# mdejong/MetalBT709Decoder

Hardware: AMD Instinct MI355X
Metric: Gpixel/s, 4k NV12->sRGB BGRA decode (output pixels) (higher is better)
Workload: dtype f32

## Files before the change

metalbt709decoder_amd/csrc/bt709_device.h:

```cpp
#pragma once

#include <hip/hip_runtime.h>

#include <cstdint>

#include "bt709_constants.h"
#include "bt709_kernels.h"
#include "bt709_quantise.h"
#include "bt709_stage.h"
#include "bt709_tile.h"

namespace bt709 {
namespace {

typedef uint32_t u32x4 __attribute__((ext_vector_type(4)));
typedef uint32_t u32x2 __attribute__((ext_vector_type(2)));
typedef __attribute__((address_space(3))) const u32x2 *LdsPairPtr;
typedef __attribute__((address_space(3))) const u32x4 *LdsQuadPtr;

__device__ __forceinline__ uint32_t lds_address(const void *p) {
  return static_cast<uint32_t>(reinterpret_cast<size_t>((__attribute__((address_space(3))) const unsigned char *)p));
}

__device__ __forceinline__ float byte_of(uint32_t w, int i) {
  float f = static_cast<float>((w >> (8 * i)) & 0xffu);
  asm("" : "+v"(f));
  return f;
}

__device__ __forceinline__ float byte_value(uint8_t b) {
  float f = static_cast<float>(b);
  asm("" : "+v"(f));
  return f;
}

__device__ __forceinline__ float centre_norm(float v, float off) {
  return __builtin_fmaf(v, kInv255, -off * kInv255);
}

__device__ __forceinline__ float add_sat(float a, float b) {
  float r;
  asm("v_add_f32_e64 %0, %1, %2 clamp" : "=v"(r) : "v"(a), "v"(b));
  return r;
}

struct Chroma {
  float cr_r, cb_g, cr_g, cb_b;
};

__device__ __forceinline__ Chroma chroma_terms(float cb, float cr) {
  const float cbn = centre_norm(cb, 128.0f);
  const float crn = centre_norm(cr, 128.0f);
  Chroma c;
  c.cr_r = __fmul_rn(crn, kMCrR);
  c.cb_g = __fmul_rn(cbn, kMCbG);
  c.cr_g = __fmul_rn(crn, kMCrG);
  c.cb_b = __fmul_rn(cbn, kMCbB);
  return c;
}

__device__ __forceinline__ void pixel_rgb(float ybyte, const Chroma &c, float &r, float &g, float &b) {
  const float yv = __fmul_rn(centre_norm(ybyte, 16.0f), kMY);
  r = add_sat(yv, c.cr_r);
  g = add_sat(__fadd_rn(yv, c.cb_g), c.cr_g);
  b = add_sat(yv, c.cb_b);
}

__device__ __forceinline__ float alpha_value(float abyte) {
  return add_sat(__fmul_rn(centre_norm(abyte, 16.0f), kMY), 0.0f);
}

__device__ __forceinline__ uint32_t quantise_byte(float x) {
  return quantise_enumerated(x);
}

__device__ __forceinline__ void magic_index12(const float *x, uint32_t *t, float magic) {
#pragma unroll
  for (int i = 0; i < 12; ++i) t[i] = __float_as_uint(__fadd_rn(x[i], magic));
}

__device__ __forceinline__ void magic_index4(const float *x, uint32_t *t, float magic) {
#pragma unroll
  for (int i = 0; i < 4; ++i) t[i] = __float_as_uint(__fadd_rn(x[i], magic));
}

struct UnitLookup {
  float magic;
  uint32_t offset;
  uint32_t shift;
};

template <typename Params>
__device__ __forceinline__ UnitLookup unit_lookup(const Params &p, const void *lds_table) {
  UnitLookup u;
  u.magic = p.unit1_magic;
  u.offset = lds_address(lds_table) - (p.unit1_first << 3);
  u.shift = p.unit1_shift;
  return u;
}

__device__ __forceinline__ uint32_t bucket_byte(const UnitLookup &u, float x, uint32_t t) {
  const u32x2 e = *reinterpret_cast<LdsPairPtr>((t << 3) + u.offset);
  return e.y + (x >= __uint_as_float(e.x) ? 1u : 0u);
}

__device__ __forceinline__ uint32_t pack_bgra(uint32_t R, uint32_t G, uint32_t B, uint32_t alpha_word) {
  const uint32_t rg = __builtin_amdgcn_perm(R, G, 0x0c04000cu);
  return rg | B | alpha_word;
}

__device__ __forceinline__ void stage_table(void *lds, const void *src, uint32_t bytes) {
  u32x4 *d = reinterpret_cast<u32x4 *>(lds);
  const u32x4 *s = reinterpret_cast<const u32x4 *>(src);
  const uint32_t tid = threadIdx.y * blockDim.x + threadIdx.x, nthreads = blockDim.x * blockDim.y;
  const uint32_t n = bytes / 16;
  if (n <= nthreads) {
    for (uint32_t i = tid; i < n; i += nthreads) d[i] = s[i];
    return;
  }
  stage_batched<5>(d, n, tid, nthreads, [&](uint32_t i) { return s[i]; });
}

template <bool NT>
__device__ __forceinline__ void store16(uint8_t *p, u32x4 v) {
  if (NT) __builtin_nontemporal_store(v, reinterpret_cast<u32x4 *>(p));
  else *reinterpret_cast<u32x4 *>(p) = v;
}

template <bool NT>
__device__ __forceinline__ void store8(uint8_t *p, u32x2 v) {
  if (NT) __builtin_nontemporal_store(v, reinterpret_cast<u32x2 *>(p));
  else *reinterpret_cast<u32x2 *>(p) = v;
}

__device__ __forceinline__ FramePlanes frame_planes(const DecodeParams &p, uint32_t i) {
  if (!p.uniform) return p.frames[i];
  FramePlanes f = p.frames[0];
  f.y += static_cast<int64_t>(i) * p.step_y;
  f.cbcr += static_cast<int64_t>(i) * p.step_cbcr;
  if (f.alpha) f.alpha += static_cast<int64_t>(i) * p.step_alpha;
  f.out += static_cast<int64_t>(i) * p.step_out;
  return f;
}

}
}
```

metalbt709decoder_amd/csrc/bt709_kernels.hip:

```cpp
#include <hip/hip_runtime.h>

#include <cstdint>
#include <cstring>

#include "bt709_device.h"
#include "bt709_launch.h"

namespace bt709 {
namespace {

template <bool HAS_ALPHA, bool QUANT, bool LOGIDX>
__device__ __forceinline__ void decode_quad(const UnitLookup &u, uint32_t ya, uint32_t yb, uint32_t cw, uint32_t aa,
                                            uint32_t ab, uint32_t alpha_word, u32x4 &top, u32x4 &bot) {
  const Chroma c0 = chroma_terms(byte_of(cw, 0), byte_of(cw, 1));
  const Chroma c1 = chroma_terms(byte_of(cw, 2), byte_of(cw, 3));
  float x[24];
#pragma unroll
  for (int px = 0; px < 8; ++px)
    pixel_rgb(byte_of(px < 4 ? ya : yb, px & 3), (px & 2) ? c1 : c0, x[3 * px], x[3 * px + 1], x[3 * px + 2]);
  static_assert(QUANT || !HAS_ALPHA, "an alpha decoder runs the sRGB mode");
  uint32_t byte[24], al[8];
  if (QUANT) {
#pragma unroll
    for (int i = 0; i < 24; ++i) byte[i] = quantise_byte(x[i]);
  } else {
    uint32_t t[24];
    magic_index12(x, t, u.magic);
    magic_index12(x + 12, t + 12, u.magic);
    if (LOGIDX) {
#pragma unroll
      for (int i = 0; i < 24; ++i) t[i] >>= 16;
    }
#pragma unroll
    for (int i = 0; i < 24; ++i) byte[i] = bucket_byte(u, x[i], t[i]);
  }
#pragma unroll
  for (int px = 0; px < 8; ++px)
    al[px] = HAS_ALPHA ? quantise_byte(alpha_value(byte_of(px < 4 ? aa : ab, px & 3))) << 24 : alpha_word;
  top.x = pack_bgra(byte[0], byte[1], byte[2], al[0]);
  top.y = pack_bgra(byte[3], byte[4], byte[5], al[1]);
  top.z = pack_bgra(byte[6], byte[7], byte[8], al[2]);
  top.w = pack_bgra(byte[9], byte[10], byte[11], al[3]);
  bot.x = pack_bgra(byte[12], byte[13], byte[14], al[4]);
  bot.y = pack_bgra(byte[15], byte[16], byte[17], al[5]);
  bot.z = pack_bgra(byte[18], byte[19], byte[20], al[6]);
  bot.w = pack_bgra(byte[21], byte[22], byte[23], al[7]);
}

template <bool HAS_ALPHA, bool QUANT>
__device__ __forceinline__ void decode_block(const UnitLookup &u, const float y[4], float cb, float cr, const float a[4],
                                             uint32_t alpha_word, uint32_t out[4]) {
  const Chroma c = chroma_terms(cb, cr);
  float x[12];
#pragma unroll
  for (int px = 0; px < 4; ++px) pixel_rgb(y[px], c, x[3 * px], x[3 * px + 1], x[3 * px + 2]);
  if (QUANT) {
#pragma unroll
    for (int px = 0; px < 4; ++px)
      out[px] = pack_bgra(quantise_byte(x[3 * px]), quantise_byte(x[3 * px + 1]), quantise_byte(x[3 * px + 2]),
                          HAS_ALPHA ? quantise_byte(alpha_value(a[px])) << 24 : alpha_word);
    return;
  }
  uint32_t t[12];
  magic_index12(x, t, u.magic);
#pragma unroll
  for (int i = 0; i < 12; ++i) t[i] >>= u.shift;
#pragma unroll
  for (int px = 0; px < 4; ++px)
    out[px] = pack_bgra(bucket_byte(u, x[3 * px], t[3 * px]), bucket_byte(u, x[3 * px + 1], t[3 * px + 1]),
                        bucket_byte(u, x[3 * px + 2], t[3 * px + 2]), alpha_word);
}

typedef __attribute__((address_space(3))) const float *LdsFloatPtr;

struct OverLookup {
  float enc_add;
  uint32_t enc_off;
  uint32_t lin_off;
};

__device__ __forceinline__ OverLookup stage_over_tables(unsigned char *lds_raw, const DecodeParams &p) {
  stage_table(lds_raw, p.table_encode, p.table_encode_bytes);
  stage_table(lds_raw + p.table_encode_bytes, p.over_table_lin, kOverLinBytes);
  OverLookup o;
  o.enc_add = p.encode_log_add;
  o.enc_off = lds_address(lds_raw) - (p.encode_log_first << 3);
  o.lin_off = lds_address(lds_raw) + p.table_encode_bytes;
  return o;
}

__device__ __forceinline__ float over_lin(const OverLookup &o, uint32_t byte) {
  return *reinterpret_cast<LdsFloatPtr>((byte << 2) + o.lin_off);
}

__device__ __forceinline__ uint32_t over_encode(const OverLookup &o, float v) {
  const uint32_t t = __float_as_uint(__fadd_rn(v, o.enc_add)) >> 16;
  const u32x2 e = *reinterpret_cast<LdsPairPtr>((t << 3) + o.enc_off);
  return e.y + (v >= __uint_as_float(e.x) ? 1u : 0u);
}

template <int OVER>
__device__ __forceinline__ uint32_t over_pixel(const OverLookup &o, const float *colour_lin, const float *x, float abyte, uint32_t bg) {
  const uint32_t as = quantise_byte(alpha_value(abyte)), inv = 255u - as;
  const float k = __fmul_rn(static_cast<float>(inv), kInv255);
  float d[3];
  uint32_t a = 255u;
  if (OVER == kOverDestination) {
    d[0] = over_lin(o, (bg >> 16) & 0xffu);
    d[1] = over_lin(o, (bg >> 8) & 0xffu);
    d[2] = over_lin(o, bg & 0xffu);
    a = as + (inv * (bg >> 24) + 127u) / 255u;
  } else {
    d[0] = colour_lin[0], d[1] = colour_lin[1], d[2] = colour_lin[2];
  }
  uint32_t byte[3];
#pragma unroll
  for (int c = 0; c < 3; ++c)
    byte[c] = over_encode(o, add_sat(over_lin(o, quantise_byte(x[c])), __fmul_rn(k, d[c])));
  return pack_bgra(byte[0], byte[1], byte[2], a << 24);
}

template <int OVER>
__device__ __forceinline__ void over_quad(const OverLookup &o, const DecodeParams &p, uint32_t ya, uint32_t yb, uint32_t cw, uint32_t aa,
                                          uint32_t ab, const u32x4 &bt, const u32x4 &bb, u32x4 &top, u32x4 &bot) {
  const Chroma c0 = chroma_terms(byte_of(cw, 0), byte_of(cw, 1));
  const Chroma c1 = chroma_terms(byte_of(cw, 2), byte_of(cw, 3));
  const uint32_t bg[8] = {bt.x, bt.y, bt.z, bt.w, bb.x, bb.y, bb.z, bb.w};
  uint32_t w[8];
#pragma unroll
  for (int px = 0; px < 8; ++px) {
    float x[3];
    pixel_rgb(byte_of(px < 4 ? ya : yb, px & 3), (px & 2) ? c1 : c0, x[0], x[1], x[2]);
    w[px] = over_pixel<OVER>(o, p.over_lin, x, byte_of(px < 4 ? aa : ab, px & 3), bg[px]);
  }
  top.x = w[0], top.y = w[1], top.z = w[2], top.w = w[3];
  bot.x = w[4], bot.y = w[5], bot.z = w[6], bot.w = w[7];
}

}

template <bool HAS_ALPHA, bool NT, bool QUANT, bool LOGIDX = false, int OVER = kOverOff>
__device__ __forceinline__ void quads_body(const DecodeParams &p, unsigned char *lds_raw) {
  constexpr int UNROLL = kQuadsPerLane;
  const BandedWork work = banded_work<true>(p.xcd_bands, p.frames_per_band);
  const FramePlanes f = frame_planes(p, work.frame);
  const uint32_t quads = p.width >> 2;
  const uint32_t row_pairs = p.height >> 1;
  const uint32_t rp_raw = blockIdx.y * blockDim.y + __builtin_amdgcn_readfirstlane(threadIdx.y);
  const uint32_t q0 = work.tile * (blockDim.x * UNROLL) + threadIdx.x;

  static_assert(OVER == kOverOff || HAS_ALPHA, "there is nothing to composite without an alpha channel");
  TileIn<UNROLL, HAS_ALPHA, OVER == kOverDestination> in;
  in.template load<NT>(f, p, rp_raw, row_pairs, q0, quads);
  OverLookup ol = {};
  if constexpr (OVER != kOverOff) {
    ol = stage_over_tables(lds_raw, p);
    __syncthreads();
  }
  if (!QUANT) {
    stage_table(lds_raw, p.table_unit, p.table_unit_bytes);
    __syncthreads();
  }
  in.pin();

  const UnitLookup ul = unit_lookup(p, lds_raw);
  uint8_t *o0 = f.out + static_cast<size_t>(2 * min(rp_raw, row_pairs - 1)) * p.out_stride;
  uint8_t *o1 = o0 + p.out_stride;
  if constexpr (OVER != kOverOff) {
#pragma unroll
    for (int u = 0; u < UNROLL; ++u) {
      const uint32_t q = q0 + u * blockDim.x;
      u32x4 top, bot;
      over_quad<OVER>(ol, p, in.ya[u], in.yb[u], in.cw[u], in.aa[u], in.ab[u], in.da[OVER == kOverDestination ? u : 0], in.db[OVER == kOverDestination ? u : 0], top, bot);
      if (q < quads && rp_raw < row_pairs) {
        store16<NT>(o0 + 16 * q, top);
        store16<NT>(o1 + 16 * q, bot);
      }
    }
    return;
  }
#pragma unroll
  for (int u = 0; u < UNROLL; ++u) {
    const uint32_t q = q0 + u * blockDim.x;
    u32x4 top, bot;
    decode_quad<HAS_ALPHA, QUANT, LOGIDX>(ul, in.ya[u], in.yb[u], in.cw[u], HAS_ALPHA ? in.aa[u] : 0u, HAS_ALPHA ? in.ab[u] : 0u, p.alpha_word, top, bot);
    if (q < quads && rp_raw < row_pairs) {
      store16<NT>(o0 + 16 * q, top);
      store16<NT>(o1 + 16 * q, bot);
    }
  }
}

template <bool HAS_ALPHA, bool NT, bool QUANT>
__global__ void __launch_bounds__(kMaxBlockThreads)
decode_nv12_quads(const DecodeParams p) {
  extern __shared__ __attribute__((aligned(16))) unsigned char lds_raw[];
  quads_body<HAS_ALPHA, NT, QUANT>(p, lds_raw);
}

template <bool NT>
__global__ void __launch_bounds__(kMaxBlockThreads)
decode_nv12_quads_log(const DecodeParams p) {
  extern __shared__ __attribute__((aligned(16))) unsigned char lds_raw[];
  quads_body<false, NT, false, true>(p, lds_raw);
}

template <int OVER>
__global__ void __launch_bounds__(kMaxBlockThreads)
decode_nv12_quads_over(const DecodeParams p) {
  extern __shared__ __attribute__((aligned(16))) unsigned char lds_raw[];
  quads_body<true, true, true, false, OVER>(p, lds_raw);
}

template <bool HAS_ALPHA, bool QUANT>
__global__ void __launch_bounds__(kBlockThreads)
decode_nv12_blocks(const DecodeParams p) {
  extern __shared__ __attribute__((aligned(16))) unsigned char lds_raw[];
  if (!QUANT) {
    stage_table(lds_raw, p.table_unit, p.table_unit_bytes);
    __syncthreads();
  }

  const UnitLookup ul = unit_lookup(p, lds_raw);
  const FramePlanes f = frame_planes(p, blockIdx.y);
  const uint32_t bw = p.width >> 1;
  const uint32_t row_pairs = p.height >> 1;

  for (uint32_t rp = blockIdx.x; rp < row_pairs; rp += gridDim.x) {
    const uint8_t *y0 = f.y + static_cast<size_t>(2 * rp) * p.y_stride;
    const uint8_t *y1 = y0 + p.y_stride;
    const uint8_t *cc = f.cbcr + static_cast<size_t>(rp) * p.cbcr_stride;
    uint32_t *o0 = reinterpret_cast<uint32_t *>(f.out + static_cast<size_t>(2 * rp) * p.out_stride);
    uint32_t *o1 = reinterpret_cast<uint32_t *>(f.out + static_cast<size_t>(2 * rp + 1) * p.out_stride);
    for (uint32_t bx = threadIdx.x; bx < bw; bx += kBlockThreads) {
      const float y[4] = {byte_value(y0[2 * bx]), byte_value(y0[2 * bx + 1]), byte_value(y1[2 * bx]),
                          byte_value(y1[2 * bx + 1])};
      float a[4] = {0.f, 0.f, 0.f, 0.f};
      if (HAS_ALPHA) {
        const uint8_t *a0 = f.alpha + static_cast<size_t>(2 * rp) * p.alpha_stride;
        const uint8_t *a1 = a0 + p.alpha_stride;
        a[0] = byte_value(a0[2 * bx]);
        a[1] = byte_value(a0[2 * bx + 1]);
        a[2] = byte_value(a1[2 * bx]);
        a[3] = byte_value(a1[2 * bx + 1]);
      }
      uint32_t out[4];
      decode_block<HAS_ALPHA, QUANT>(ul, y, byte_value(cc[2 * bx]), byte_value(cc[2 * bx + 1]), a, p.alpha_word, out);
      o0[2 * bx] = out[0];
      o0[2 * bx + 1] = out[1];
      o1[2 * bx] = out[2];
      o1[2 * bx + 1] = out[3];
    }
  }
}

template <int OVER>
__global__ void __launch_bounds__(kBlockThreads)
decode_nv12_blocks_over(const DecodeParams p) {
  extern __shared__ __attribute__((aligned(16))) unsigned char lds_raw[];
  const OverLookup ol = stage_over_tables(lds_raw, p);
  __syncthreads();

  const FramePlanes f = frame_planes(p, blockIdx.y);
  const uint32_t bw = p.width >> 1;
  const uint32_t row_pairs = p.height >> 1;

  for (uint32_t rp = blockIdx.x; rp < row_pairs; rp += gridDim.x) {
    const uint8_t *y0 = f.y + static_cast<size_t>(2 * rp) * p.y_stride;
    const uint8_t *y1 = y0 + p.y_stride;
    const uint8_t *a0 = f.alpha + static_cast<size_t>(2 * rp) * p.alpha_stride;
    const uint8_t *a1 = a0 + p.alpha_stride;
    const uint8_t *cc = f.cbcr + static_cast<size_t>(rp) * p.cbcr_stride;
    uint32_t *o0 = reinterpret_cast<uint32_t *>(f.out + static_cast<size_t>(2 * rp) * p.out_stride);
    uint32_t *o1 = reinterpret_cast<uint32_t *>(f.out + static_cast<size_t>(2 * rp + 1) * p.out_stride);
    for (uint32_t bx = threadIdx.x; bx < bw; bx += kBlockThreads) {
      const float y[4] = {byte_value(y0[2 * bx]), byte_value(y0[2 * bx + 1]), byte_value(y1[2 * bx]), byte_value(y1[2 * bx + 1])};
      const float a[4] = {byte_value(a0[2 * bx]), byte_value(a0[2 * bx + 1]), byte_value(a1[2 * bx]), byte_value(a1[2 * bx + 1])};
      uint32_t bg[4] = {0u, 0u, 0u, 0u};
      if (OVER == kOverDestination) bg[0] = o0[2 * bx], bg[1] = o0[2 * bx + 1], bg[2] = o1[2 * bx], bg[3] = o1[2 * bx + 1];
      const Chroma c = chroma_terms(byte_value(cc[2 * bx]), byte_value(cc[2 * bx + 1]));
      uint32_t out[4];
#pragma unroll
      for (int px = 0; px < 4; ++px) {
        float x[3];
        pixel_rgb(y[px], c, x[0], x[1], x[2]);
        out[px] = over_pixel<OVER>(ol, p.over_lin, x, a[px], bg[px]);
      }
      o0[2 * bx] = out[0];
      o0[2 * bx + 1] = out[1];
      o1[2 * bx] = out[2];
      o1[2 * bx + 1] = out[3];
    }
  }
}

struct UnconvertParams {
  const uint8_t *in;
  uint8_t *out;
  int64_t in_step, out_step;
  const uint8_t *ins[kMaxBatch];
  uint8_t *outs[kMaxBatch];
  uint32_t use_table;
  uint32_t in_stride, out_stride, width, height;
  const void *table_unit;
  uint32_t table_unit_bytes;
  float unit1_magic;
  uint32_t unit1_first, unit1_shift;
  uint32_t alpha_word;
};

template <bool VEC, bool QUANT>
__global__ void __launch_bounds__(kBlockThreads)
unconvert_packed444(const UnconvertParams p) {
  extern __shared__ __attribute__((aligned(16))) unsigned char lds_raw[];
  constexpr uint32_t N = VEC ? 4 : 1, ROWS = VEC ? 2 : 1;
  const uint32_t row0 = blockIdx.y * ROWS;
  const uint32_t i = blockIdx.x * blockDim.x + threadIdx.x;
  const uint8_t *frame_in = p.use_table ? p.ins[blockIdx.z] : p.in + static_cast<int64_t>(blockIdx.z) * p.in_step;
  uint8_t *frame_out = p.use_table ? p.outs[blockIdx.z] : p.out + static_cast<int64_t>(blockIdx.z) * p.out_step;
  const bool live = i * N < p.width;
  const uint32_t ic = live ? i : 0u;
  uint32_t w[ROWS][N];
#pragma unroll
  for (uint32_t r = 0; r < ROWS; ++r) {
    const uint8_t *in = frame_in + static_cast<size_t>(row0 + r) * p.in_stride;
    if (VEC) {
      const u32x4 v = __builtin_nontemporal_load(reinterpret_cast<const u32x4 *>(in + 16 * ic));
      w[r][0] = v.x, w[r][N > 1 ? 1 : 0] = v.y, w[r][N > 2 ? 2 : 0] = v.z, w[r][N > 3 ? 3 : 0] = v.w;
    } else {
      w[r][0] = *reinterpret_cast<const uint32_t *>(in + 4 * ic);
    }
  }
  if (!QUANT) {
    stage_table(lds_raw, p.table_unit, p.table_unit_bytes);
    __syncthreads();
  }
  const UnitLookup ul = unit_lookup(p, lds_raw);
  if (!live) return;
#pragma unroll
  for (uint32_t r = 0; r < ROWS; ++r) {
    float x[3 * N];
#pragma unroll
    for (uint32_t k = 0; k < N; ++k) {
      const Chroma c = chroma_terms(byte_of(w[r][k], 1), byte_of(w[r][k], 2));
      pixel_rgb(byte_of(w[r][k], 0), c, x[3 * k], x[3 * k + 1], x[3 * k + 2]);
    }
    uint32_t o[N];
#pragma unroll
    for (uint32_t k = 0; k < N; ++k) {
      uint32_t b[3];
#pragma unroll
      for (int ch = 0; ch < 3; ++ch)
        b[ch] = QUANT ? quantise_byte(x[3 * k + ch]) : bucket_byte(ul, x[3 * k + ch], __float_as_uint(__fadd_rn(x[3 * k + ch], ul.magic)) >> ul.shift);
      o[k] = pack_bgra(b[0], b[1], b[2], p.alpha_word);
    }
    uint8_t *out = frame_out + static_cast<size_t>(row0 + r) * p.out_stride;
    if (VEC) {
      u32x4 v;
      v.x = o[0], v.y = o[N > 1 ? 1 : 0], v.z = o[N > 2 ? 2 : 0], v.w = o[N > 3 ? 3 : 0];
      __builtin_nontemporal_store(v, reinterpret_cast<u32x4 *>(out + 16 * i));
    } else {
      *reinterpret_cast<uint32_t *>(out + 4 * i) = o[0];
    }
  }
}

const char *launch_unconvert(const DecodeParams &t, const UnconvertBatch &b, size_t in_stride, size_t out_stride, uint32_t width, uint32_t height,
                             bool vec, bool quantiser, hipStream_t stream) {
  UnconvertParams p;
  std::memset(&p, 0, sizeof p);
  p.in = static_cast<const uint8_t *>(b.in[0]);
  p.out = static_cast<uint8_t *>(b.out[0]);
  p.in_step = b.in_step;
  p.out_step = b.out_step;
  p.use_table = b.uniform ? 0u : 1u;
  if (!b.uniform)
    for (int i = 0; i < b.count && i < kMaxBatch; ++i) p.ins[i] = static_cast<const uint8_t *>(b.in[i]), p.outs[i] = static_cast<uint8_t *>(b.out[i]);
  p.in_stride = static_cast<uint32_t>(in_stride);
  p.out_stride = static_cast<uint32_t>(out_stride);
  p.width = width;
  p.height = height;
  p.table_unit = t.table_unit;
  p.table_unit_bytes = t.table_unit_bytes;
  p.unit1_magic = t.unit1_magic;
  p.unit1_first = t.unit1_first;
  p.unit1_shift = t.unit1_shift;
  p.alpha_word = t.alpha_word;
  const uint32_t groups = vec ? width / 4 : width;
  const dim3 grid((groups + kBlockThreads - 1) / kBlockThreads, vec ? height / 2 : height, static_cast<uint32_t>(b.count));
  const size_t lds = quantiser ? 0 : t.table_unit_bytes;
  if (vec) {
    if (quantiser) hipLaunchKernelGGL((unconvert_packed444<true, true>), grid, dim3(kBlockThreads), lds, stream, p);
    else hipLaunchKernelGGL((unconvert_packed444<true, false>), grid, dim3(kBlockThreads), lds, stream, p);
  } else {
    if (quantiser) hipLaunchKernelGGL((unconvert_packed444<false, true>), grid, dim3(kBlockThreads), lds, stream, p);
    else hipLaunchKernelGGL((unconvert_packed444<false, false>), grid, dim3(kBlockThreads), lds, stream, p);
  }
  return vec ? "unconvert_packed444<vec>" : "unconvert_packed444";
}

LaunchShape &last_launch_shape() {
  static thread_local LaunchShape shape = {};
  return shape;
}

const char *launch_decode(const DecodeParams &p_in, int frames, int variant, bool has_alpha, bool quantiser, bool nontemporal,
                          int xcd_bands, uint32_t grid_x, uint32_t block_threads, hipStream_t stream) {
  const bool quant = quantiser || has_alpha;
  const uint32_t over = has_alpha ? p_in.over_mode : kOverOff;
  const size_t lds = over != kOverOff ? p_in.table_encode_bytes + kOverLinBytes : (quant ? 0 : p_in.table_unit_bytes);
  const BandPlan plan = plan_bands(frames, variant == kVariantQuads && xcd_bands, p_in.uniform, kXcdBandMinFrames);
  if (plan.banded && plan.tail) {
    launch_decode(p_in, plan.banded, variant, has_alpha, quantiser, nontemporal, xcd_bands, grid_x, block_threads, stream);
    DecodeParams tail = p_in;
    advance_frames(tail, plan.banded);
    return launch_decode(tail, plan.tail, variant, has_alpha, quantiser, nontemporal, 0, grid_x, block_threads, stream);
  }
  DecodeParams p = p_in;
  if (variant == kVariantQuads) {
    const uint32_t by = quads_rows_per_block(block_threads, grid_x);
    dim3 grid(grid_x, (p.height / 2 + by - 1) / by, static_cast<uint32_t>(frames));
    const dim3 block(block_threads, by, 1);
    if (plan.banded) grid = band_grid(p, static_cast<uint32_t>(xcd_bands), grid);
    record_launch(grid, block, p.xcd_bands);
    if (over == kOverDestination) {
      hipLaunchKernelGGL((decode_nv12_quads_over<kOverDestination>), grid, block, lds, stream, p);
      return "decode_nv12_quads<alpha,over>";
    }
    if (over != kOverOff) {
      hipLaunchKernelGGL((decode_nv12_quads_over<kOverColour>), grid, block, lds, stream, p);
      return "decode_nv12_quads<alpha,over-colour>";
    }
    if (has_alpha) {
      hipLaunchKernelGGL((decode_nv12_quads<true, true, true>), grid, block, lds, stream, p);
      return "decode_nv12_quads<alpha>";
    }
    if (quant) {
      if (nontemporal) hipLaunchKernelGGL((decode_nv12_quads<false, true, true>), grid, block, lds, stream, p);
      else hipLaunchKernelGGL((decode_nv12_quads<false, false, true>), grid, block, lds, stream, p);
      return nontemporal ? "decode_nv12_quads<nt,quantiser>" : "decode_nv12_quads<quantiser>";
    }
    if (p_in.unit1_shift != 0) {
      if (nontemporal) hipLaunchKernelGGL((decode_nv12_quads_log<true>), grid, block, lds, stream, p);
      else hipLaunchKernelGGL((decode_nv12_quads_log<false>), grid, block, lds, stream, p);
      return nontemporal ? "decode_nv12_quads_log<nt>" : "decode_nv12_quads_log";
    }
    if (nontemporal) {
      hipLaunchKernelGGL((decode_nv12_quads<false, true, false>), grid, block, lds, stream, p);
      return "decode_nv12_quads<nt>";
    }
    hipLaunchKernelGGL((decode_nv12_quads<false, false, false>), grid, block, lds, stream, p);
    return "decode_nv12_quads";
  }
  const dim3 grid(grid_x, static_cast<uint32_t>(frames), 1);
  const dim3 block(kBlockThreads, 1, 1);
  record_launch(grid, block, 0);
  if (over == kOverDestination) {
    hipLaunchKernelGGL((decode_nv12_blocks_over<kOverDestination>), grid, block, lds, stream, p);
    return "decode_nv12_blocks<alpha,over>";
  }
  if (over != kOverOff) {
    hipLaunchKernelGGL((decode_nv12_blocks_over<kOverColour>), grid, block, lds, stream, p);
    return "decode_nv12_blocks<alpha,over-colour>";
  }
  if (has_alpha) {
    hipLaunchKernelGGL((decode_nv12_blocks<true, true>), grid, block, lds, stream, p);
    return "decode_nv12_blocks<alpha>";
  }
  if (quant) {
    hipLaunchKernelGGL((decode_nv12_blocks<false, true>), grid, block, lds, stream, p);
    return "decode_nv12_blocks<quantiser>";
  }
  hipLaunchKernelGGL((decode_nv12_blocks<false, false>), grid, block, lds, stream, p);
  return "decode_nv12_blocks";
}

hipError_t prepare_kernels() {
  const void *fns[] = {
      reinterpret_cast<const void *>(&decode_nv12_quads<true, true, true>),
      reinterpret_cast<const void *>(&decode_nv12_quads<false, true, true>),
      reinterpret_cast<const void *>(&decode_nv12_quads<false, false, true>),
      reinterpret_cast<const void *>(&decode_nv12_quads<false, true, false>),
      reinterpret_cast<const void *>(&decode_nv12_quads<false, false, false>),
      reinterpret_cast<const void *>(&decode_nv12_quads_log<true>),
      reinterpret_cast<const void *>(&decode_nv12_quads_log<false>),
      reinterpret_cast<const void *>(&unconvert_packed444<true, false>),
      reinterpret_cast<const void *>(&unconvert_packed444<false, false>),
      reinterpret_cast<const void *>(&decode_nv12_blocks<true, true>),
      reinterpret_cast<const void *>(&decode_nv12_blocks<false, true>),
      reinterpret_cast<const void *>(&decode_nv12_blocks<false, false>),
  };
  return raise_lds_cap(fns, kRepLdsBytes);
}

}
```

metalbt709decoder_amd/csrc/bt709_tile.h:

```cpp
#pragma once

#include <hip/hip_runtime.h>

#include <cstdint>

#include "bt709_kernels.h"

namespace bt709 {
namespace {

struct BandedWork {
  uint32_t tile, frame;
};
template <bool INTERLEAVED = false>
__device__ __forceinline__ BandedWork banded_work(uint32_t xcd_bands, uint32_t frames_per_band) {
  const uint32_t band = blockIdx.x & 7u;
  BandedWork w;
  w.tile = xcd_bands ? blockIdx.x >> 3 : blockIdx.x;
  if (INTERLEAVED) w.frame = xcd_bands == 1 ? band * frames_per_band + blockIdx.z : (xcd_bands == 2 ? blockIdx.z * 8u + band : blockIdx.z);
  else w.frame = xcd_bands ? band * frames_per_band + blockIdx.z : blockIdx.z;
  return w;
}

template <bool NT>
__device__ __forceinline__ uint32_t load32(const uint8_t *p) {
  if (NT) return __builtin_nontemporal_load(reinterpret_cast<const uint32_t *>(p));
  return *reinterpret_cast<const uint32_t *>(p);
}

typedef uint32_t TileWord16 __attribute__((ext_vector_type(4)));
template <int N, bool HAS_ALPHA, bool DEST = false>
struct TileIn {
  uint32_t ya[N], yb[N], cw[N], aa[N], ab[N];
  TileWord16 da[DEST ? N : 1], db[DEST ? N : 1];

  template <bool NT>
  __device__ __forceinline__ void load(const FramePlanes &f, const DecodeParams &p, uint32_t rp, uint32_t row_pairs, uint32_t q0, uint32_t quads) {
    rp = min(rp, row_pairs - 1);
    const uint8_t *y0 = f.y + static_cast<size_t>(2 * rp) * p.y_stride;
    const uint8_t *y1 = y0 + p.y_stride;
    const uint8_t *cc = f.cbcr + static_cast<size_t>(rp) * p.cbcr_stride;
    const uint8_t *a0 = HAS_ALPHA ? f.alpha + static_cast<size_t>(2 * rp) * p.alpha_stride : nullptr;
#pragma unroll
    for (int j = 0; j < N; ++j) {
      const uint32_t q = min(q0 + j * blockDim.x, quads - 1);
      ya[j] = load32<NT>(y0 + 4 * q);
      yb[j] = load32<NT>(y1 + 4 * q);
      cw[j] = load32<NT>(cc + 4 * q);
      if (HAS_ALPHA) {
        aa[j] = load32<NT>(a0 + 4 * q);
        ab[j] = load32<NT>(a0 + p.alpha_stride + 4 * q);
      }
      if (DEST) {
        const uint8_t *o0 = f.out + static_cast<size_t>(2 * rp) * p.out_stride + 16 * static_cast<size_t>(q);
        da[DEST ? j : 0] = __builtin_nontemporal_load(reinterpret_cast<const TileWord16 *>(o0));
        db[DEST ? j : 0] = __builtin_nontemporal_load(reinterpret_cast<const TileWord16 *>(o0 + p.out_stride));
      }
    }
  }

  __device__ __forceinline__ void pin() {
#pragma unroll
    for (int j = 0; j < N; ++j) {
      asm volatile("" : "+v"(ya[j]), "+v"(yb[j]), "+v"(cw[j]));
      if (HAS_ALPHA) asm volatile("" : "+v"(aa[j]), "+v"(ab[j]));
      if (DEST) asm volatile("" : "+v"(da[DEST ? j : 0]), "+v"(db[DEST ? j : 0]));
    }
  }
};

}
}
```

metalbt709decoder_amd/csrc/transfer_tables.cpp:

```cpp
#include "transfer_tables.h"

#include <cfenv>
#include <cmath>
#include <cstring>
#include <limits>

namespace bt709 {

float srgb_to_linear(float v) {
  if (v <= 0.04045f) return v * (1.0f / 12.92f);
  const float a = 0.055f;
  const float gamma = 2.4f;
  const float base = (v + a) * (1.0f / (1.0f + a));
  return static_cast<float>(std::pow(static_cast<double>(base), static_cast<double>(gamma)));
}

float linear_to_srgb(float v) {
  if (v <= 0.0031308f) return v * 12.92f;
  const float a = 0.055f;
  const float gamma = 1.0f / 2.4f;
  const double r = static_cast<double>(1.0f + a) *
                       std::pow(static_cast<double>(v), static_cast<double>(gamma)) -
                   static_cast<double>(a);
  return static_cast<float>(r);
}

float itu709_to_linear(float v) {
  if (v < 0.081f) return v * (1.0f / 4.5f);
  const float a = 0.099f;
  const float gamma = 1.0f / 0.45f;
  const float base = (v + a) * (1.0f / (1.0f + a));
  return static_cast<float>(std::pow(static_cast<double>(base), static_cast<double>(gamma)));
}

float apple196_to_linear(float v) {
  const float x_intercept = 0.05583828f;
  if (v < x_intercept) return v * (1.0f / 16.0f);
  const float gamma = 1.960938f;
  return static_cast<float>(std::pow(static_cast<double>(v), static_cast<double>(gamma)));
}

float linear_to_apple196(float v) {
  const float y_intercept = 0.00349f;
  if (v < y_intercept) return v * 16.0f;
  const float gamma = 1.0f / 1.960938f;
  return static_cast<float>(std::pow(static_cast<double>(v), static_cast<double>(gamma)));
}

int quantize_byte(float v) {
  const float scaled = v * 255.0f;
  return static_cast<int>(std::round(static_cast<double>(scaled)));
}

int transfer_to_byte(int gamma, float v) {
  switch (gamma) {
    case kGammaApple:
      return quantize_byte(linear_to_srgb(apple196_to_linear(v)));
    case kGammaSRGB:
      return quantize_byte(v);
    case kGammaLinear:
      return quantize_byte(linear_to_srgb(v));
    case kGammaITU709:
      return quantize_byte(linear_to_srgb(itu709_to_linear(v)));
    case kTableEncodeApple:
      return quantize_byte(linear_to_apple196(v));
    default:
      return -1;
  }
}

namespace {

float from_bits(uint32_t u) {
  float f;
  std::memcpy(&f, &u, sizeof f);
  return f;
}

float find_threshold(int gamma, int k) {
  uint32_t lo = 0, hi = 0x3f800000u;
  if (transfer_to_byte(gamma, from_bits(hi)) < k) return std::numeric_limits<float>::infinity();
  while (lo < hi) {
    const uint32_t mid = lo + (hi - lo) / 2;
    if (transfer_to_byte(gamma, from_bits(mid)) >= k) hi = mid;
    else lo = mid + 1;
  }
  return from_bits(lo);
}

uint32_t to_bits(float f) {
  uint32_t u;
  std::memcpy(&u, &f, sizeof u);
  return u;
}

}

uint32_t bucket_index(float x, float magic) {
  volatile float s = x + magic;
  return to_bits(s) - to_bits(magic);
}

bool build_transfer_table(int gamma, TransferTable *out) {
  if (gamma < 0 || gamma >= kTableKinds || out == nullptr) return false;
  out->gamma = gamma;
  for (int k = 1; k <= 255; ++k) out->thresholds[k - 1] = find_threshold(gamma, k);

  float lin_of_byte[257];
  for (int b = 0; b < 256; ++b) lin_of_byte[b] = srgb_to_linear(b * (1.0f / 255.0f));
  lin_of_byte[256] = lin_of_byte[255];

  const float inf = std::numeric_limits<float>::infinity();
  for (uint32_t n = 256; n <= 65536; n *= 2) {
    const float magic = 8388608.0f / static_cast<float>(n);
    std::vector<TransferBucket> b(n + 1, TransferBucket{inf, 0u});
    bool ok = true;
    std::vector<uint32_t> held(n + 2, 0u);
    for (int k = 0; k < 255 && ok; ++k) {
      if (out->thresholds[k] == inf) continue;
      const uint32_t q = bucket_index(out->thresholds[k], magic);
      if (q > n || held[q] != 0) ok = false;
      else held[q] = 1, b[q].edge = out->thresholds[k];
    }
    if (!ok) continue;
    uint32_t before = 0;
    for (uint32_t q = 0; q <= n; ++q) {
      b[q].base = before;
      before += held[q];
    }
    out->n = n;
    out->buckets_unit = b;
    while ((out->buckets_unit.size() * sizeof(TransferBucket)) % 16 != 0)
      out->buckets_unit.push_back(TransferBucket{inf, 255u});
    out->buckets_linear.resize(b.size());
    for (size_t q = 0; q < b.size(); ++q) {
      TransferBucketLinear &e = out->buckets_linear[q];
      e.edge_pred = b[q].edge == inf ? inf : std::nextafter(b[q].edge, -inf);
      e.base = b[q].base;
      e.lin_below = std::ldexp(lin_of_byte[b[q].base], kLinearScaleLog2);
      e.lin_above = std::ldexp(lin_of_byte[b[q].base + 1], kLinearScaleLog2);
    }
    out->log_add = 0.0f;
    out->log_first = 0;
    out->buckets_log.clear();
    for (int e = 3; e <= 10; ++e) {
      const float add = std::ldexp(1.0f, -e);
      const uint32_t first = bucket_index_log(0.0f, add), count = bucket_index_log(1.0f, add) - first + 1;
      if (2 * count > n + 1) break;
      std::vector<TransferBucket> lb(count, TransferBucket{inf, 0u});
      std::vector<uint32_t> lheld(count, 0u);
      bool fits = true;
      for (int k = 0; k < 255 && fits; ++k) {
        if (out->thresholds[k] == inf) continue;
        const uint32_t q = bucket_index_log(out->thresholds[k], add) - first;
        if (q >= count || lheld[q] != 0) fits = false;
        else lheld[q] = 1, lb[q].edge = out->thresholds[k];
      }
      if (!fits) continue;
      uint32_t seen = 0;
      for (uint32_t q = 0; q < count; ++q) {
        lb[q].base = seen;
        seen += lheld[q];
      }
      out->log_add = add;
      out->log_first = first;
      out->buckets_log = lb;
      while ((out->buckets_log.size() * sizeof(TransferBucket)) % 16 != 0) out->buckets_log.push_back(TransferBucket{inf, 255u});
      break;
    }
    return true;
  }
  return false;
}

uint32_t bucket_index_log(float x, float log_add) {
  volatile float t = x + log_add;
  return to_bits(t) >> 16;
}

uint16_t float_to_half(float v) {
  const uint32_t u = to_bits(v), sign = (u >> 16) & 0x8000u;
  const uint32_t a = u & 0x7fffffffu;
  if (a >= 0x7f800000u) return static_cast<uint16_t>(sign | 0x7c00u | ((a > 0x7f800000u) ? 0x200u : 0u));
  if (a >= 0x477ff000u) return static_cast<uint16_t>(sign | 0x7c00u);
  if (a < 0x33000001u) return static_cast<uint16_t>(sign);
  const int exp = static_cast<int>(a >> 23) - 127;
  uint32_t mant = (a & 0x7fffffu) | 0x800000u;
  int shift;
  uint32_t base;
  if (exp >= -14) {
    shift = 13;
    base = static_cast<uint32_t>(exp + 15 - 1) << 10;
  } else {
    shift = 13 + (-14 - exp);
    base = 0;
  }
  const uint32_t kept = mant >> shift, rest = mant & ((1u << shift) - 1u), half_ulp = 1u << (shift - 1);
  uint32_t h = base + kept;
  if (rest > half_ulp || (rest == half_ulp && (kept & 1u))) ++h;
  return static_cast<uint16_t>(sign | h);
}

float curve_to_linear(int gamma, float v) {
  switch (gamma) {
    case kGammaApple: return apple196_to_linear(v);
    case kGammaSRGB: return srgb_to_linear(v);
    case kGammaITU709: return itu709_to_linear(v);
    default: return v;
  }
}

bool build_half_table(int gamma, HalfTable *out) {
  if (gamma < 0 || gamma >= kGammaCount || out == nullptr) return false;
  const float inf = std::numeric_limits<float>::infinity();
  out->gamma = gamma;
  out->pre_add = 0.0f;
  out->pre_scale = 1.0f;
  out->exponent = 1.0f;
  out->low_scale = 1.0f;
  out->thresholds.clear();
  switch (gamma) {
    case kGammaApple:
      out->split = 0.05583828f;
      out->low_scale = 1.0f / 16.0f;
      out->exponent = 1.960938f;
      break;
    case kGammaSRGB:
      out->split = std::nextafter(0.04045f, 1.0f);
      out->low_scale = 1.0f / 12.92f;
      out->pre_add = 0.055f;
      out->pre_scale = 1.0f / (1.0f + 0.055f);
      out->exponent = 2.4f;
      break;
    case kGammaITU709:
      out->split = 0.081f;
      out->low_scale = 1.0f / 4.5f;
      out->pre_add = 0.099f;
      out->pre_scale = 1.0f / (1.0f + 0.099f);
      out->exponent = 1.0f / 0.45f;
      break;
    default:
      out->split = 2.0f;
      out->h_min = 0;
      out->thresholds.assign(4, inf);
      return true;
  }
  auto H = [gamma](float x) { return static_cast<uint32_t>(float_to_half(curve_to_linear(gamma, x))); };
  const uint32_t lo_bits = to_bits(out->split), hi_bits = 0x3f800000u;
  out->h_min = H(out->split);
  const uint32_t h_max = H(1.0f);
  {
    uint32_t lo = 0, hi = lo_bits;
    while (lo < hi) {
      const uint32_t mid = lo + (hi - lo) / 2;
      if (H(from_bits(mid)) >= out->h_min) hi = mid;
      else lo = mid + 1;
    }
    out->thresholds.push_back(from_bits(lo));
  }
  for (uint32_t h = out->h_min + 1; h <= h_max; ++h) {
    uint32_t lo = lo_bits, hi = hi_bits;
    while (lo < hi) {
      const uint32_t mid = lo + (hi - lo) / 2;
      if (H(from_bits(mid)) >= h) hi = mid;
      else lo = mid + 1;
    }
    out->thresholds.push_back(from_bits(lo));
  }
  out->thresholds.push_back(inf);
  while (out->thresholds.size() % 4 != 0) out->thresholds.push_back(inf);
  {
    const float edge = 0.0625f, below = std::nextafter(out->split, 0.0f);
    const uint32_t s0 = to_bits(edge / out->split);
    bool found = false;
    for (int d = 0; d <= 16 && !found; ++d) {
      for (int sign = -1; sign <= 1 && !found; sign += 2) {
        const float s = from_bits(s0 + static_cast<uint32_t>(sign * d));
        volatile float at = out->split * s, under = below * s;
        if (at >= edge && under < edge) {
          out->index_scale = s;
          found = true;
        }
      }
    }
    if (!found) return false;
  }
  out->cand.clear();
  out->cand.push_back(0.0f);
  out->cand.push_back(out->low_scale);
  const double a = out->pre_add, s = out->pre_scale, g = out->exponent, keep = 1.0 - 1.0 / 524288.0;
  const float ninf = -std::numeric_limits<float>::infinity();
  const uint32_t last = half_cand_index(*out, 1.0f);
  uint32_t start = lo_bits;
  for (uint32_t i = 1; i <= last; ++i) {
    uint32_t lo = start, hi = hi_bits;
    while (lo < hi) {
      const uint32_t mid = lo + (hi - lo) / 2;
      if (half_cand_index(*out, from_bits(mid)) >= i) hi = mid;
      else lo = mid + 1;
    }
    start = lo;
    const double xq = from_bits(lo);
    const double base = (xq + a) * s;
    const double value = std::pow(base, g) * keep, slope = g * s * std::pow(base, g - 1.0) * keep;
    out->cand.push_back(std::nextafter(static_cast<float>(value - slope * xq), ninf));
    out->cand.push_back(std::nextafter(static_cast<float>(slope), ninf));
  }
  if (half_cand_index(*out, out->split) != 1 || half_cand_index(*out, std::nextafter(out->split, 0.0f)) != 0) return false;
  return true;
}

uint32_t half_cand_index(const HalfTable &t, float x) {
  volatile float u = x * t.index_scale;
  const uint32_t ub = to_bits(u);
  uint32_t hb = ub >= (113u << 23) ? (ub - (112u << 23)) >> 13 : 0u;
  if (hb < kHalfCandFloor) hb = kHalfCandFloor;
  return (hb >> 3) - (kHalfCandFloor >> 3);
}

float half_candidate(const HalfTable &t, float x) {
  if (t.cand.empty() || !(x >= 0.0f && x <= 1.0f)) return 0.0f;
  const uint32_t i = half_cand_index(t, x);
  volatile float p = std::fmaf(x, t.cand[2 * i + 1], t.cand[2 * i]);
  return p;
}

uint32_t uniform_index(float v, float n) {
  volatile float t = std::fmaf(v, n, 8388608.0f);
  return to_bits(t) - 0x4b000000u;
}

bool build_uniform_table(int kind, uint32_t n_min, UniformTable *out) {
  if (kind < 0 || kind >= kTableKinds || out == nullptr) return false;
  float thr[255];
  for (int k = 1; k <= 255; ++k) thr[k - 1] = find_threshold(kind, k);
  const float inf = std::numeric_limits<float>::infinity();
  for (uint32_t n = (n_min + 31) / 32 * 32; n <= 65536; n += 32) {
    const float nf = static_cast<float>(n);
    std::vector<TransferBucket> b(n + 2, TransferBucket{inf, 0u});
    std::vector<uint32_t> held(n + 2, 0u);
    bool ok = true;
    for (int k = 0; k < 255 && ok; ++k) {
      if (thr[k] == inf) continue;
      const uint32_t q = uniform_index(thr[k], nf);
      if (q > n + 1 || held[q] != 0) ok = false;
      else held[q] = 1, b[q].edge = thr[k];
    }
    if (!ok || uniform_index(1.0f, nf) > n + 1) continue;
    uint32_t before = 0;
    for (uint32_t q = 0; q < n + 2; ++q) {
      b[q].base = before;
      before += held[q];
    }
    while ((b.size() * sizeof(TransferBucket)) % 16 != 0) b.push_back(TransferBucket{inf, 255u});
    out->n = n;
    out->buckets = b;
    return true;
  }
  return false;
}

bool build_split_table(int kind, SplitTable *out) {
  if (kind < 0 || kind >= kTableKinds || out == nullptr) return false;
  float thr[255];
  for (int k = 1; k <= 255; ++k) thr[k - 1] = find_threshold(kind, k);
  const float inf = std::numeric_limits<float>::infinity();
  const struct { uint32_t n_fine, split, ratio; } cand[] = {
      {256, 256, 1},   {512, 512, 1},   {1024, 64, 4},  {2048, 128, 4},  {4096, 256, 8},
      {4096, 256, 4},  {4096, 512, 4},  {8192, 512, 8}, {8192, 1024, 4}, {4096, 4096, 1}, {8192, 8192, 1}};
  for (const auto &c : cand) {
    const uint32_t coarse_n = c.n_fine / c.ratio;
    const uint32_t offset = c.split - c.split / c.ratio;
    const uint32_t total = c.split + (coarse_n - c.split / c.ratio) + 1;
    std::vector<TransferBucket> b(total);
    bool ok = true;
    int k = 0;
    for (uint32_t q = 0; q < total && ok; ++q) {
      float lo, hi;
      if (q < c.split) {
        lo = static_cast<float>(q) / c.n_fine;
        hi = static_cast<float>(q + 1) / c.n_fine;
      } else {
        const uint32_t j = q - offset;
        lo = static_cast<float>(j) / coarse_n;
        hi = static_cast<float>(j + 1) / coarse_n;
      }
      while (k < 255 && thr[k] <= lo) ++k;
      b[q].base = static_cast<uint32_t>(k);
      b[q].edge = inf;
      if (k < 255 && thr[k] < hi) {
        b[q].edge = thr[k] * static_cast<float>(c.n_fine);
        if (k + 1 < 255 && thr[k + 1] < hi) ok = false;
      }
    }
    if (!ok) continue;
    while ((b.size() * sizeof(TransferBucket)) % 16 != 0) b.push_back(TransferBucket{inf, 255u});
    out->n_fine = c.n_fine;
    out->split = static_cast<float>(c.split);
    out->coarse_scale = 1.0f / static_cast<float>(c.ratio);
    out->coarse_offset = offset;
    out->buckets = b;
    return true;
  }
  return false;
}

bool build_encode_tables(int in_gamma, int out_gamma, EncodeTables *out) {
  if (out == nullptr) return false;
  auto ok = [](int g) { return g == kGammaApple || g == kGammaSRGB || g == kGammaLinear; };
  if (!ok(in_gamma) || !ok(out_gamma)) return false;
  out->from_linear_kind = out_gamma == kGammaSRGB ? kGammaLinear : (out_gamma == kGammaLinear ? kGammaSRGB : kTableEncodeApple);
  for (int b = 0; b < 256; ++b) {
    const float n = b * (1.0f / 255.0f);
    float lin = n;
    if (in_gamma == kGammaSRGB) lin = srgb_to_linear(n);
    else if (in_gamma == kGammaApple) lin = apple196_to_linear(n);
    const int e = transfer_to_byte(out->from_linear_kind, lin);
    out->per_byte[b].lin = lin;
    out->per_byte[b].enc_norm = e * (1.0f / 255.0f);
  }
  return true;
}

}
```

Before: 1167.

## Prefetch LUT tables before tile loads and fuse log-bucket address computation

Table words are now fetched from global memory into registers before the tile's input loads are issued, and written to LDS afterwards. This lets the table fetch latency overlap with the pixel loads. The log-index bucket address is computed with a single v_mad_u32_u16 on the high half instead of a shift followed by a shift-and-add. The host rule for choosing a log table is changed to compare its padded byte size against the unit table, and the pin order is reversed when tables are staged. The combined fetch relies on the table fitting in one word per thread. Otherwise it falls back to batched staging, which reloads from global memory.

```diff
diff --git a/metalbt709decoder_amd/csrc/bt709_device.h b/metalbt709decoder_amd/csrc/bt709_device.h
--- a/metalbt709decoder_amd/csrc/bt709_device.h
+++ b/metalbt709decoder_amd/csrc/bt709_device.h
@@ -109,6 +109,42 @@
   return rg | B | alpha_word;
 }
 
+__device__ __forceinline__ uint32_t log_bucket_address(uint32_t t, uint32_t offset) {
+  uint32_t a;
+  asm("v_mad_u32_u16 %0, %1, 8, %2 op_sel:[1,0,0,0]" : "=v"(a) : "v"(t), "s"(offset));
+  return a;
+}
+
+__device__ __forceinline__ uint32_t bucket_byte_log(const UnitLookup &u, float x, uint32_t t) {
+  const u32x2 e = *reinterpret_cast<LdsPairPtr>(log_bucket_address(t, u.offset));
+  return e.y + (x >= __uint_as_float(e.x) ? 1u : 0u);
+}
+
+struct TableFetch {
+  u32x4 word;
+};
+
+__device__ __forceinline__ TableFetch fetch_table(const void *src, uint32_t bytes) {
+  const u32x4 *s = reinterpret_cast<const u32x4 *>(src);
+  const uint32_t tid = threadIdx.y * blockDim.x + threadIdx.x, nthreads = blockDim.x * blockDim.y;
+  const uint32_t n = bytes / 16;
+  TableFetch f = {};
+  if (n - 1u < nthreads) f.word = s[min(tid, n - 1u)];
+  return f;
+}
+
+__device__ __forceinline__ void commit_table(void *lds, const void *src, uint32_t bytes, const TableFetch &f) {
+  u32x4 *d = reinterpret_cast<u32x4 *>(lds);
+  const u32x4 *s = reinterpret_cast<const u32x4 *>(src);
+  const uint32_t tid = threadIdx.y * blockDim.x + threadIdx.x, nthreads = blockDim.x * blockDim.y;
+  const uint32_t n = bytes / 16;
+  if (n <= nthreads) {
+    if (tid < n) d[tid] = f.word;
+    return;
+  }
+  stage_batched<5>(d, n, tid, nthreads, [&](uint32_t i) { return s[i]; });
+}
+
 __device__ __forceinline__ void stage_table(void *lds, const void *src, uint32_t bytes) {
   u32x4 *d = reinterpret_cast<u32x4 *>(lds);
   const u32x4 *s = reinterpret_cast<const u32x4 *>(src);
diff --git a/metalbt709decoder_amd/csrc/bt709_kernels.hip b/metalbt709decoder_amd/csrc/bt709_kernels.hip
--- a/metalbt709decoder_amd/csrc/bt709_kernels.hip
+++ b/metalbt709decoder_amd/csrc/bt709_kernels.hip
@@ -27,12 +27,8 @@
     uint32_t t[24];
     magic_index12(x, t, u.magic);
     magic_index12(x + 12, t + 12, u.magic);
-    if (LOGIDX) {
-#pragma unroll
-      for (int i = 0; i < 24; ++i) t[i] >>= 16;
-    }
-#pragma unroll
-    for (int i = 0; i < 24; ++i) byte[i] = bucket_byte(u, x[i], t[i]);
+#pragma unroll
+    for (int i = 0; i < 24; ++i) byte[i] = LOGIDX ? bucket_byte_log(u, x[i], t[i]) : bucket_byte(u, x[i], t[i]);
   }
 #pragma unroll
   for (int px = 0; px < 8; ++px)
@@ -79,14 +75,35 @@
   uint32_t lin_off;
 };
 
-__device__ __forceinline__ OverLookup stage_over_tables(unsigned char *lds_raw, const DecodeParams &p) {
-  stage_table(lds_raw, p.table_encode, p.table_encode_bytes);
-  stage_table(lds_raw + p.table_encode_bytes, p.over_table_lin, kOverLinBytes);
+__device__ __forceinline__ OverLookup over_lookup(const unsigned char *lds_raw, const DecodeParams &p) {
   OverLookup o;
   o.enc_add = p.encode_log_add;
   o.enc_off = lds_address(lds_raw) - (p.encode_log_first << 3);
   o.lin_off = lds_address(lds_raw) + p.table_encode_bytes;
   return o;
+}
+
+__device__ __forceinline__ OverLookup stage_over_tables(unsigned char *lds_raw, const DecodeParams &p) {
+  stage_table(lds_raw, p.table_encode, p.table_encode_bytes);
+  stage_table(lds_raw + p.table_encode_bytes, p.over_table_lin, kOverLinBytes);
+  return over_lookup(lds_raw, p);
+}
+
+struct OverFetch {
+  TableFetch enc, lin;
+};
+
+__device__ __forceinline__ OverFetch fetch_over_tables(const DecodeParams &p) {
+  OverFetch f;
+  f.enc = fetch_table(p.table_encode, p.table_encode_bytes);
+  f.lin = fetch_table(p.over_table_lin, kOverLinBytes);
+  return f;
+}
+
+__device__ __forceinline__ OverLookup commit_over_tables(unsigned char *lds_raw, const DecodeParams &p, const OverFetch &f) {
+  commit_table(lds_raw, p.table_encode, p.table_encode_bytes, f.enc);
+  commit_table(lds_raw + p.table_encode_bytes, p.over_table_lin, kOverLinBytes, f.lin);
+  return over_lookup(lds_raw, p);
 }
 
 __device__ __forceinline__ float over_lin(const OverLookup &o, uint32_t byte) {
@@ -150,18 +167,22 @@
   const uint32_t q0 = work.tile * (blockDim.x * UNROLL) + threadIdx.x;
 
   static_assert(OVER == kOverOff || HAS_ALPHA, "there is nothing to composite without an alpha channel");
+  OverFetch over_fetch = {};
+  TableFetch unit_fetch = {};
+  if constexpr (OVER != kOverOff) over_fetch = fetch_over_tables(p);
+  if (!QUANT) unit_fetch = fetch_table(p.table_unit, p.table_unit_bytes);
   TileIn<UNROLL, HAS_ALPHA, OVER == kOverDestination> in;
   in.template load<NT>(f, p, rp_raw, row_pairs, q0, quads);
   OverLookup ol = {};
   if constexpr (OVER != kOverOff) {
-    ol = stage_over_tables(lds_raw, p);
+    ol = commit_over_tables(lds_raw, p, over_fetch);
     __syncthreads();
   }
   if (!QUANT) {
-    stage_table(lds_raw, p.table_unit, p.table_unit_bytes);
+    commit_table(lds_raw, p.table_unit, p.table_unit_bytes, unit_fetch);
     __syncthreads();
   }
-  in.pin();
+  in.template pin<!QUANT || OVER != kOverOff>();
 
   const UnitLookup ul = unit_lookup(p, lds_raw);
   uint8_t *o0 = f.out + static_cast<size_t>(2 * min(rp_raw, row_pairs - 1)) * p.out_stride;
diff --git a/metalbt709decoder_amd/csrc/bt709_tile.h b/metalbt709decoder_amd/csrc/bt709_tile.h
--- a/metalbt709decoder_amd/csrc/bt709_tile.h
+++ b/metalbt709decoder_amd/csrc/bt709_tile.h
@@ -59,9 +59,11 @@
     }
   }
 
+  template <bool LAST_FIRST = false>
   __device__ __forceinline__ void pin() {
 #pragma unroll
-    for (int j = 0; j < N; ++j) {
+    for (int i = 0; i < N; ++i) {
+      const int j = LAST_FIRST ? N - 1 - i : i;
       asm volatile("" : "+v"(ya[j]), "+v"(yb[j]), "+v"(cw[j]));
       if (HAS_ALPHA) asm volatile("" : "+v"(aa[j]), "+v"(ab[j]));
       if (DEST) asm volatile("" : "+v"(da[DEST ? j : 0]), "+v"(db[DEST ? j : 0]));
diff --git a/metalbt709decoder_amd/csrc/transfer_tables.cpp b/metalbt709decoder_amd/csrc/transfer_tables.cpp
--- a/metalbt709decoder_amd/csrc/transfer_tables.cpp
+++ b/metalbt709decoder_amd/csrc/transfer_tables.cpp
@@ -146,7 +146,8 @@
     for (int e = 3; e <= 10; ++e) {
       const float add = std::ldexp(1.0f, -e);
       const uint32_t first = bucket_index_log(0.0f, add), count = bucket_index_log(1.0f, add) - first + 1;
-      if (2 * count > n + 1) break;
+      const size_t padded = (count * sizeof(TransferBucket) + 15) / 16 * 16;
+      if (padded >= out->buckets_unit.size() * sizeof(TransferBucket)) break;
       std::vector<TransferBucket> lb(count, TransferBucket{inf, 0u});
       std::vector<uint32_t> lheld(count, 0u);
       bool fits = true;
```

New measurement: 1165. No clear change (-0.2%).
